# lemma-osu/sknnr

Hardware: AMD Instinct MI355X
Metric: Mqueries/sec + achieved HBM GB/s, 10M×50k×32 k=5, 1/2/4/8 MI355X (higher is better)
Workload: dtype f16 split MFMA (hi.hi swept, lo.hi + hi.lo corrections; f32 accumulate) pre-filter + f64 exact re-score

## Files before the change

sknnr_amd/csrc/bucket.hip.h:

```cpp
#pragma once
#include <hip/hip_runtime.h>
#include <stdint.h>

namespace sknnr {

constexpr int kCellMaxDepth = 6;
constexpr int kCellMax = 1 << kCellMaxDepth;
constexpr int kBucketBlock = 1024;
#ifndef SKNNR_BUCKET_CHUNKS
#define SKNNR_BUCKET_CHUNKS 32
#endif
constexpr int kBucketChunks = SKNNR_BUCKET_CHUNKS;

struct CellTreeDev {
    const float* axes;
    const float* centre;
    const float* thr;
    int depth;
};

__device__ __forceinline__ int cell_of(const float (&z)[kCellMaxDepth], const CellTreeDev& t) {
    int node = 0;
#pragma unroll
    for (int l = 0; l < kCellMaxDepth; ++l)
        if (l < t.depth) node = 2 * node + (z[l] >= t.thr[(1 << l) - 1 + node] ? 1 : 0);
    return node;
}

struct CellArgs {
    const double* xq;
    long nq;
    long n_pad;
    int d;
    int depth;
    const float* axes;
    const float* centre;
    const float* thr;
    unsigned char* cell;
    int* hist;
    int* perm;
    const double* qnc;
    double* qnc_pos;
};

#ifdef SKNNR_KERNELS_EXACT
__global__ void __launch_bounds__(256) cell_assign_kernel(CellArgs a) {
    const long q = (long)blockIdx.x * 256 + threadIdx.x;
    if (q < a.nq) {
        const double* row = a.xq + q * a.d;
        float z[kCellMaxDepth];
#pragma unroll
        for (int l = 0; l < kCellMaxDepth; ++l) z[l] = 0.f;
        auto feed = [&](int k, double x) {
            const float v = (float)x - a.centre[k];
#pragma unroll
            for (int l = 0; l < kCellMaxDepth; ++l)
                if (l < a.depth) z[l] = fmaf(v, a.axes[l * a.d + k], z[l]);
        };
        int k = 0;
        if ((a.d & 3) == 0) {
            const double2* r2 = (const double2*)row;
            for (; k + 8 <= a.d; k += 8) {
                const double2 v0 = r2[k / 2], v1 = r2[k / 2 + 1], v2 = r2[k / 2 + 2], v3 = r2[k / 2 + 3];
                feed(k, v0.x); feed(k + 1, v0.y); feed(k + 2, v1.x); feed(k + 3, v1.y);
                feed(k + 4, v2.x); feed(k + 5, v2.y); feed(k + 6, v3.x); feed(k + 7, v3.y);
            }
        }
        for (; k < a.d; ++k) feed(k, row[k]);
        const CellTreeDev t{a.axes, a.centre, a.thr, a.depth};
        a.cell[q] = (unsigned char)cell_of(z, t);
    }
}
#endif

#ifdef SKNNR_KERNELS_EXACT
__global__ void __launch_bounds__(kBucketBlock) cell_count_kernel(CellArgs a) {
    __shared__ int h[kCellMax];
    if (threadIdx.x < kCellMax) h[threadIdx.x] = 0;
    __syncthreads();
#pragma unroll
    for (int r = 0; r < kBucketChunks; ++r) {
        const long q = ((long)blockIdx.x * kBucketChunks + r) * kBucketBlock + threadIdx.x;
        if (q < a.nq) atomicAdd(&h[a.cell[q]], 1);
    }
    __syncthreads();
    if (threadIdx.x < kCellMax && h[threadIdx.x] != 0) atomicAdd(&a.hist[threadIdx.x], h[threadIdx.x]);
}
#endif


#ifdef SKNNR_KERNELS_EXACT
__global__ void __launch_bounds__(kBucketBlock) cell_scatter_kernel(CellArgs a) {
    __shared__ int cnt[kCellMax], base[kCellMax], first[kCellMax];
    const int n_cells = 1 << a.depth;
    if (threadIdx.x < kCellMax) cnt[threadIdx.x] = 0;
    if (threadIdx.x == 0) {
        int acc = 0;
        for (int c = 0; c < kCellMax; ++c) {
            first[c] = acc;
            acc += c < n_cells ? a.hist[c] : 0;
        }
    }
    __syncthreads();
    int c[kBucketChunks], ticket[kBucketChunks];
#pragma unroll
    for (int r = 0; r < kBucketChunks; ++r) {
        const long q = ((long)blockIdx.x * kBucketChunks + r) * kBucketBlock + threadIdx.x;
        c[r] = 0;
        ticket[r] = 0;
        if (q < a.nq) {
            c[r] = a.cell[q];
            ticket[r] = atomicAdd(&cnt[c[r]], 1);
        } else if (q < a.n_pad) {
            a.perm[q] = (int)q;
            if (a.qnc_pos) a.qnc_pos[q] = a.qnc[q];
            a.cell[q] = (unsigned char)(n_cells - 1);
        }
    }
    __syncthreads();
    if (threadIdx.x < kCellMax && cnt[threadIdx.x] != 0) base[threadIdx.x] = atomicAdd(&a.hist[kCellMax + threadIdx.x], cnt[threadIdx.x]);
    __syncthreads();
#pragma unroll
    for (int r = 0; r < kBucketChunks; ++r) {
        const long q = ((long)blockIdx.x * kBucketChunks + r) * kBucketBlock + threadIdx.x;
        if (q < a.nq) {
            const int p = first[c[r]] + base[c[r]] + ticket[r];
            a.perm[p] = (int)q;
            if (a.qnc_pos) a.qnc_pos[p] = a.qnc[q];
        }
    }
}
#endif

}
```

sknnr_amd/csrc/k_exact.hip:

```cpp
#define SKNNR_KERNELS_EXACT 1
#include <cstdint>
#include <cstdlib>

#include "launch.hip.h"

namespace sknnr {
namespace {
__global__ void add_counter_kernel(const int* __restrict__ cnt, long long* __restrict__ total) { *total += *cnt; }

template <int BT>
hipError_t prep_lds_bt(const PrepArgs& a, hipStream_t st) {
    const size_t sh = (size_t)BT * (a.d_in | 1) * 8;
    hipError_t e = hipFuncSetAttribute((const void*)prep_queries_kernel<BT>, hipFuncAttributeMaxDynamicSharedMemorySize, (int)sh);
    if (e != hipSuccess) return e;
    prep_queries_kernel<BT><<<dim3((unsigned)(a.nq_pad / BT)), dim3(BT), sh, st>>>(a);
    return hipGetLastError();
}

template <int FORMULA>
hipError_t exact_scan_f(bool chunked, const ScanArgs& a, long blocks, size_t sh, hipStream_t st) {
    auto kern = chunked ? exact_scan_kernel<FORMULA, true> : exact_scan_kernel<FORMULA, false>;
    hipError_t e = hipFuncSetAttribute((const void*)kern, hipFuncAttributeMaxDynamicSharedMemorySize, (int)sh);
    if (e != hipSuccess) return e;
    kern<<<dim3((unsigned)blocks), dim3(kScanWaves * 64), sh, st>>>(a);
    return hipGetLastError();
}
}

namespace launch {

hipError_t row_norms(const double* x, long n, int d, double* out, hipStream_t st) {
    row_norms_kernel<<<dim3((unsigned)((n + 255) / 256)), dim3(256), 0, st>>>(x, n, d, out);
    return hipGetLastError();
}

template <int KS>
hipError_t prep_direct_ks(PrepArgs a, hipStream_t st) {
    a.lds_wave_bytes = prep_direct_wave_lds(KS, a.xt != nullptr, a.qimg != nullptr);
    const size_t sh = (size_t)4 * a.lds_wave_bytes;
    hipError_t e = hipFuncSetAttribute((const void*)prep_queries_direct_kernel<KS>, hipFuncAttributeMaxDynamicSharedMemorySize, (int)sh);
    if (e != hipSuccess) return e;
    prep_queries_direct_kernel<KS><<<dim3((unsigned)(a.nq_pad / 256)), dim3(256), sh, st>>>(a);
    return hipGetLastError();
}

hipError_t prep_direct(const PrepArgs& a, hipStream_t st) {
    switch (a.ks) {
        case 1: return prep_direct_ks<1>(a, st);
        case 2: return prep_direct_ks<2>(a, st);
        case 3: return prep_direct_ks<3>(a, st);
        case 4: return prep_direct_ks<4>(a, st);
    }
    return hipErrorInvalidValue;
}

hipError_t prep_lds(int rows_per_block, const PrepArgs& a, hipStream_t st) {
    switch (rows_per_block) {
        case 256: return prep_lds_bt<256>(a, st);
        case 128: return prep_lds_bt<128>(a, st);
        case 64: return prep_lds_bt<64>(a, st);
    }
    return hipErrorInvalidValue;
}

hipError_t check_finite(const double* x, long n_el, int* status, hipStream_t st) {
    const long blocks = n_el + 255 < 256L * 256 * 16 ? (n_el + 255) / 256 : 256L * 16;
    check_finite_kernel<<<dim3((unsigned)(blocks < 1 ? 1 : blocks)), dim3(256), 0, st>>>(x, n_el, status);
    return hipGetLastError();
}

hipError_t cell_assign(const CellArgs& a, hipStream_t st) {
    cell_assign_kernel<<<dim3((unsigned)((a.nq + 255) / 256)), dim3(256), 0, st>>>(a);
    return hipGetLastError();
}
hipError_t cell_count(const CellArgs& a, hipStream_t st) {
    cell_count_kernel<<<dim3((unsigned)((a.nq + kBucketBlock * kBucketChunks - 1) / (kBucketBlock * kBucketChunks))), dim3(kBucketBlock), 0, st>>>(a);
    return hipGetLastError();
}
hipError_t cell_scatter(const CellArgs& a, hipStream_t st) {
    cell_scatter_kernel<<<dim3((unsigned)((a.n_pad + kBucketBlock * kBucketChunks - 1) / (kBucketBlock * kBucketChunks))), dim3(kBucketBlock), 0, st>>>(a);
    return hipGetLastError();
}

int finalize_lanes(const FinalizeArgs& f) { return f.rec ? kRecordLen : (f.m_list <= 8 ? 16 : (f.m_list <= 16 ? 32 : 64)); }

hipError_t finalize(const FinalizeArgs& f, long n, hipStream_t st) {
    if (f.rec) {
        finalize_record_kernel<<<dim3((unsigned)((n * kRecordLen + 255) / 256)), dim3(256), finalize_lds_bytes(kRecordLen / 2, f.s.d), st>>>(f);
    } else if (f.m_list <= 8) {
        finalize_kernel<8><<<dim3((unsigned)((n * 16 + 255) / 256)), dim3(256), finalize_lds_bytes(8, f.s.d), st>>>(f);
    } else if (f.m_list <= 16) {
        finalize_kernel<16><<<dim3((unsigned)((n * 32 + 255) / 256)), dim3(256), finalize_lds_bytes(16, f.s.d), st>>>(f);
    } else {
        finalize_kernel<32><<<dim3((unsigned)((n * 64 + 255) / 256)), dim3(256), finalize_lds_bytes(32, f.s.d), st>>>(f);
    }
    return hipGetLastError();
}

hipError_t exact_scan(int formula, bool chunked, const ScanArgs& a, long blocks, size_t lds_bytes, hipStream_t st) {
    switch (formula) {
        case 0: return exact_scan_f<0>(chunked, a, blocks, lds_bytes, st);
        case 1: return exact_scan_f<1>(chunked, a, blocks, lds_bytes, st);
        default: return exact_scan_f<2>(chunked, a, blocks, lds_bytes, st);
    }
}

hipError_t scan_merge(int formula, const ScanArgs& a, long blocks, size_t lds_bytes, int grid_wg_of_scan, int forced_slices,
                      hipStream_t st) {
    const dim3 grid((unsigned)blocks), block(256);
    switch (formula) {
        case 0: scan_merge_kernel<0><<<grid, block, lds_bytes, st>>>(a, grid_wg_of_scan, forced_slices); break;
        case 1: scan_merge_kernel<1><<<grid, block, lds_bytes, st>>>(a, grid_wg_of_scan, forced_slices); break;
        default: scan_merge_kernel<2><<<grid, block, lds_bytes, st>>>(a, grid_wg_of_scan, forced_slices); break;
    }
    return hipGetLastError();
}

hipError_t pack_shards(const double* val, const long* idx, long nq, int n_shards, int kk, double* slice_v, int* slice_i,
                       hipStream_t st) {
    const long heaps = nq * n_shards * kk;
    const long blocks = (heaps + 255) / 256 < 256L * 32 ? (heaps + 255) / 256 : 256L * 32;
    pack_shards_kernel<<<dim3((unsigned)(blocks < 1 ? 1 : blocks)), dim3(256), 0, st>>>(val, idx, nq, n_shards, kk, slice_v, slice_i);
    return hipGetLastError();
}

hipError_t predict(const PredictArgs& a, hipStream_t st) {
    const long total = a.nq * a.t;
    if ((a.mode == 0 && a.y32) || (a.mode == 2 && a.w32))
        predict32_kernel<<<dim3((unsigned)((total + 255) / 256)), dim3(256), 0, st>>>(a);
    else if (a.k <= 8)
        predict_kernel<<<dim3((unsigned)((total + 255) / 256)), dim3(256), 0, st>>>(a);
    else
        predict_wide_kernel<<<dim3((unsigned)((total + 255) / 256)), dim3(256), 0, st>>>(a);
// ... 39 lines not shown
```

sknnr_amd/csrc/launch.hip.h:

```cpp
#pragma once
#include <hip/hip_runtime.h>

#include <algorithm>

#include "bucket.hip.h"
#include "coarse2.hip.h"
#include "exact.hip.h"
#include "forest.hip.h"
#include "hamming.hip.h"
#include "mask.hip.h"
#include "narrow.hip.h"
#include "planes.hip.h"
#include "rescue.hip.h"
#include "summary.hip.h"

namespace sknnr {
namespace launch {

hipError_t row_norms(const double* x, long n, int d, double* out, hipStream_t st);
hipError_t prep_direct(const PrepArgs& a, hipStream_t st);
hipError_t prep_lds(int rows_per_block, const PrepArgs& a, hipStream_t st);
hipError_t check_finite(const double* x, long n_el, int* status, hipStream_t st);
hipError_t cell_assign(const CellArgs& a, hipStream_t st);
hipError_t cell_count(const CellArgs& a, hipStream_t st);
hipError_t cell_scatter(const CellArgs& a, hipStream_t st);
hipError_t finalize(const FinalizeArgs& f, long n, hipStream_t st);
int finalize_lanes(const FinalizeArgs& f);
hipError_t exact_scan(int formula, bool chunked, const ScanArgs& a, long blocks, size_t lds_bytes, hipStream_t st);
hipError_t scan_merge(int formula, const ScanArgs& a, long blocks, size_t lds_bytes, int grid_wg_of_scan, int forced_slices,
                      hipStream_t st);
hipError_t pack_shards(const double* val, const long* idx, long nq, int n_shards, int kk, double* slice_v, int* slice_i,
                       hipStream_t st);
hipError_t predict(const PredictArgs& a, hipStream_t st);
hipError_t crosswalk(const long* table, const long* idx, long n, long* out, hipStream_t st);
hipError_t add_counter(const int* cnt, long long* total, hipStream_t st);
hipError_t rescue(int ks, const RescueArgs& a, hipStream_t st);
hipError_t rescue_account(const int* listed, const int* state, long long* total, hipStream_t st);

hipError_t hamming_pack(const double* xq, long nq, long nq_pad, int t, int tp, uint32_t* qimg, int* q_bad, hipStream_t st);
hipError_t hamming_rows(const double* x, long n, int t, int tpr, uint32_t* rows, hipStream_t st);
hipError_t hamming_coarse(const HammingArgs& a, hipStream_t st);
hipError_t hamming_rescore(const HammingRescoreArgs& a, hipStream_t st);
hipError_t hamming_distance_rows(const HammingRowsArgs& a, hipStream_t st);

hipError_t forest_apply(const ForestArgs& a, hipStream_t st);

hipError_t row_mask(const MaskArgs& a, long* n_valid, hipStream_t st);
hipError_t row_compact(const CompactArgs& a, size_t row_bytes, hipStream_t st);
int compact_unit(const void* x, const void* out, size_t row_bytes);
hipError_t row_expand(const ExpandArgs& a, hipStream_t st);

hipError_t planes_to_rows(const PlanesArgs& a, int elem_bytes, hipStream_t st);
hipError_t rows_to_planes(const PlanesArgs& a, hipStream_t st);

hipError_t narrow(const NarrowArgs& a, int kind, int dst_dtype, bool wide, hipStream_t st);
int narrow_dst_bytes(int kind, int dst_dtype);

hipError_t summary(const SummaryArgs& a, hipStream_t st);

struct Coarse1Launch {
    const char* rimg;
    int n_stages;
    const uint4* qimg;
    const double* qnc;
    float skip_scale;
    int n_sentinel;
    float* cand_val;
    int* cand_idx;
    long nq_pad;
};
struct Coarse2Launch {
    const char* rhi;
    const char* rlo;
    int n_stages;
    const uint4* qimg;
    const double* qnc;
    float skip_scale;
// ... 21 lines not shown
```

sknnr_amd/csrc/sknnr_hip.hip:

```cpp
#include "../../include/sknnr_hip.h"

#include <hip/hip_runtime.h>
#include <sys/mman.h>

#include <algorithm>
#include <chrono>
#include <cmath>
#include <cstdarg>
#include <cstdio>
#include <cstdlib>
#include <condition_variable>
#include <cstring>
#include <deque>
#include <functional>
#include <future>
#include <limits>
#include <memory>
#include <mutex>
#include <new>
#include <string>
#include <thread>
#include <vector>

#include "launch.hip.h"
// ... 181 lines not shown
                q_.pop_front();
            }
            task();
        }
    }
    std::mutex m_;
    std::condition_variable cv_;
    std::deque<std::packaged_task<int()>> q_;
    bool stop_ = false;
    std::thread th_;
};

struct sknnr_index {
    int device = 0;
    long n_ref = 0;
    int d = 0, t = 0;
    int ks = 0;
    int n_stages = 0;
    double s = 1.0;
    double ymax = 0.0;
    double mu_norm = 0.0;
    std::vector<double> mu;
    std::mutex mtx;

    int d_in = 0;
    bool has_affine = false;
    DevBuf<double> center, scale, proj;
    bool has_center = false, has_scale = false, has_proj = false;

    bool has_forest = false;
    int f_d_in = 0;
    DevBuf<int4> f_nodes;
    DevBuf<long> f_off;
    DevBuf<int> f_depth;
    DevBuf<double> f_ids;

    DevBuf<double> hw;
    double hw_sum = 0.0;
    bool has_hw = false;
    bool h16_ok = false;
    int h_tp = 0, h_ref_pad = 0;
    DevBuf<uint32_t> h_rimg, h_wq, h_qimg, h_rrow;
    DevBuf<int> h_bad, h_cand_cnt, h_cand_id;
    DevBuf<double> ref64, refT, rn64, y64, mu_dev;
    DevBuf<char> rimg;
    DevBuf<char> rhi2, rlo2;
    int n_stages2 = 0;
    DevBuf<int> perm;
    DevBuf<int> perm2;
    int cell_depth = 0;
    DevBuf<float> cell_axes, cell_centre, cell_thr;
    DevBuf<int> cell_stage;
    DevBuf<unsigned char> qcell;
    DevBuf<int> qperm, cell_hist;

    DevBuf<double> xt, qnc, xstage, dist_stage, pred_stage;
    DevBuf<uint4> qimg;
    DevBuf<float> cand_val;
    DevBuf<int> cand_idx, fail_list, fail_count, fail_list2, slice_i;
    DevBuf<unsigned long long> rec;
    DevBuf<float> rec_bound;
    DevBuf<double> qnc_pos;
    DevBuf<double> slice_v;
    DevBuf<float> fail_thr;
    DevBuf<int> resc_list, resc_state;
    bool rescue_enabled = true;
    int64_t last_rescue[2] = {};
    DevBuf<int> status;
    DevBuf<long long> fail_total;
    DevBuf<long> idx_stage;

    struct HostSlot {
        double* pin_x = nullptr;  size_t pin_x_n = 0;
        double* pin_d = nullptr;  size_t pin_d_n = 0;
        long* pin_i = nullptr;    size_t pin_i_n = 0;
        double* pin_p = nullptr;  size_t pin_p_n = 0;
        DevBuf<double> dev_x, dev_d, dev_p;
        DevBuf<long> dev_i;
        DevBuf<double> dev_xp, dev_dp, dev_pp;
        DevBuf<long> dev_ip;
        DevBuf<unsigned long long> nar_i, nar_d, nar_p;
        hipEvent_t ev_h2d = nullptr, ev_done = nullptr, ev_d2h = nullptr;
        MaskBufs mask;
    } slot[kHostSlots];
    hipStream_t st_h2d = nullptr, st_run = nullptr, st_d2h = nullptr;
    std::unique_ptr<HostWorker> w_in, w_out;

    hipEvent_t ev_ws = nullptr;
    bool ws_busy = false;
    hipStream_t st_side = nullptr;
    hipEvent_t ev_fork = nullptr, ev_join = nullptr;
    long bulk_rows_done = 0;
    hipEvent_t ev_bulk_end = nullptr;
    int64_t last_prefilter[8] = {};
    int64_t last_finalize[2] = {};
    int64_t last_hamming[8] = {};
    long last_hamming_rows = 0;
    int64_t last_scan[8] = {};
    int64_t last_prep[8] = {};
    const double* last_prep_xt = nullptr;
    bool last_prep_bucketed = false, last_prep_qnc_pos = false;
    bool stream_open = false;
    MaskBufs mask;
    DevBuf<double> m_nodata, s_nodata;
    int64_t last_mask[8] = {};
    int64_t last_planes[8] = {};
    DevBuf<double> s_scale, s_offset;
    int64_t last_narrow[8] = {};
    const SummaryPlan* summary = nullptr;
    DevBuf<int> c_stat, s_stat;
    int64_t last_summary[8] = {};

    struct CallTiming {
        hipEvent_t e0 = nullptr, e1 = nullptr;
        std::vector<std::pair<hipEvent_t, hipEvent_t>> coarse;
        size_t coarse_used = 0;
        long coarse_rows = 0;
        bool pending = false;
    };
    static constexpr int kTimingRing = 64;
    CallTiming timing[kTimingRing];
    int timing_next = 0;
    sknnr_stats stats{};

    ~sknnr_index() {
        w_in.reset();
        w_out.reset();
        (void)hipSetDevice(device);
        for (auto* b : {&center, &scale, &proj, &ref64, &refT, &rn64, &y64, &mu_dev, &xt, &qnc, &xstage,
                        &dist_stage, &pred_stage, &f_ids})
            b->release();
        f_nodes.release(); f_off.release(); f_depth.release();
        rimg.release();
        perm.release();
        perm2.release();
        cell_axes.release(); cell_centre.release(); cell_thr.release(); cell_stage.release();
        qcell.release(); qperm.release(); cell_hist.release();
        h_rimg.release(); h_wq.release(); h_qimg.release(); h_rrow.release(); h_bad.release(); h_cand_cnt.release(); h_cand_id.release();
        qimg.release();
        cand_val.release();
        cand_idx.release();
        rec.release(); rec_bound.release(); qnc_pos.release();
        fail_list.release();
        fail_count.release();
        fail_thr.release(); resc_list.release(); resc_state.release();
        fail_total.release();
        status.release();
        idx_stage.release();
        for (auto& sl : slot) {
            for (void* hp : {(void*)sl.pin_x, (void*)sl.pin_d, (void*)sl.pin_i, (void*)sl.pin_p})
                if (hp) (void)hipHostFree(hp);
            sl.dev_x.release(); sl.dev_d.release(); sl.dev_p.release(); sl.dev_i.release();
            sl.dev_xp.release(); sl.dev_dp.release(); sl.dev_pp.release(); sl.dev_ip.release();
            sl.nar_i.release(); sl.nar_d.release(); sl.nar_p.release();
            for (hipEvent_t e : {sl.ev_h2d, sl.ev_done, sl.ev_d2h})
                if (e) (void)hipEventDestroy(e);
        }
        for (hipStream_t h : {st_h2d, st_run, st_d2h})
            if (h) (void)hipStreamDestroy(h);
        if (ev_ws) (void)hipEventDestroy(ev_ws);
        if (st_side) (void)hipStreamDestroy(st_side);
        for (hipEvent_t e : {ev_fork, ev_join})
            if (e) (void)hipEventDestroy(e);
        for (auto& ct : timing) {
            for (hipEvent_t e : {ct.e0, ct.e1})
                if (e) (void)hipEventDestroy(e);
            for (auto& pr : ct.coarse) {
                (void)hipEventDestroy(pr.first);
                (void)hipEventDestroy(pr.second);
            }
        }
    }
};

extern "C" int32_t sknnr_device_count(void) {
    int n = 0;
    if (hipGetDeviceCount(&n) != hipSuccess) return 0;
    return n;
}

extern "C" int32_t sknnr_abi_version(void) { return SKNNR_ABI_VERSION; }

extern "C" const char* sknnr_last_error(void) { return g_last_error.c_str(); }

extern "C" int sknnr_index_shape(const sknnr_index* ix, int64_t* n_ref, int32_t* d, int32_t* t,
                                 int32_t* d_in, int32_t* device) {
    if (!ix) return fail(SKNNR_ERR_INVALID, "index is NULL");
    if (n_ref) *n_ref = ix->n_ref;
    if (d) *d = ix->d;
    if (t) *t = ix->t;
    if (d_in) *d_in = ix->has_affine ? ix->d_in : (ix->has_forest ? ix->f_d_in : ix->d);
    if (device) *device = ix->device;
    return SKNNR_OK;
}

static bool mahalanobis_norms(const double* ref, int64_t n_ref, int d, const std::vector<double>& mu,
                              std::vector<double>& out) {
    if ((double)n_ref * d * d > 8e9 || n_ref < 2 * (int64_t)d) return false;
// ... 404 lines not shown
                    std::vector<int> first_s((size_t)n_cells + 1, sim.S);
                    for (int pos = sim.S - 1; pos >= 0; --pos) first_s[(size_t)tree.code[(size_t)by_cell[(size_t)pos]]] = pos;
                    for (int c = n_cells - 1; c >= 0; --c)
                        if (first_s[(size_t)c] == sim.S) first_s[(size_t)c] = first_s[(size_t)c + 1];
                    const int window = std::max<int>(32, (int)((int64_t)seed_tiles_for(n_tiles2, tps2) * 32 * sim.S / n_ref));
                    std::vector<int> start((size_t)sim.NQ);
                    for (int qi = 0; qi < sim.NQ; ++qi) {
                        int node = 0;
                        for (int l = 0; l < depth; ++l) {
                            float z = 0.f;
                            for (int k = 0; k < d; ++k)
                                z = std::fmaf((float)sim.q[(size_t)qi * d + k] - tree.centre[(size_t)k], tree.axes[(size_t)l * d + k], z);
                            node = 2 * node + (z >= tree.thr[((size_t)1 << l) - 1 + node] ? 1 : 0);
                        }
                        const int mid = (first_s[(size_t)node] + first_s[(size_t)node + 1]) / 2;
                        start[(size_t)qi] = ((mid - window / 2) % sim.S + sim.S) % sim.S;
                    }
                    const long v_cell = sim.visits(by_cell, &start);
                    if (v_cell * 100 >= order_visits * 85) depth = 0;
                    if (std::getenv("SKNNR_ORDER_TRACE"))
                        std::fprintf(stderr, "[order] best plain order %d: %ld visits; cell order (depth %d): %ld visits -> %s\n", image_order,
                                     order_visits, tree.depth, v_cell, depth ? "cells" : "plain");
                }
            }
            if (depth > 0) {
                for (int64_t i = 0; i < n_ref; ++i) perm2[(size_t)i] = (int)i;
                const bool by_norm = std::getenv("SKNNR_CELL_NORM_ORDER") != nullptr;
                std::stable_sort(perm2.begin(), perm2.end(), [&](int a, int b) {
                    if (tree.code[(size_t)a] != tree.code[(size_t)b]) return tree.code[(size_t)a] < tree.code[(size_t)b];
                    if (by_norm) return cnorm[(size_t)a] < cnorm[(size_t)b];
                    return mix((uint32_t)a) < mix((uint32_t)b);
                });
                const int n_cells = 1 << depth;
                std::vector<long> first((size_t)n_cells + 1, n_ref);
                for (int64_t pos = n_ref - 1; pos >= 0; --pos) first[(size_t)tree.code[(size_t)perm2[(size_t)pos]]] = pos;
                for (int c = n_cells - 1; c >= 0; --c)
                    if (first[(size_t)c] == n_ref) first[(size_t)c] = first[(size_t)c + 1];
                std::vector<int> stage((size_t)n_cells);
                for (int c = 0; c < n_cells; ++c) {
                    const long mid_tile = (first[(size_t)c] + first[(size_t)c + 1]) / 2 / 32;
                    const long half = seed_tiles_for(n_tiles2, tps2) / 2;
                    long st = (mid_tile - half) / tps2;
                    if (mid_tile - half < 0) st = ix->n_stages2 + (mid_tile - half - tps2 + 1) / tps2;
                    stage[(size_t)c] = (int)(((st % ix->n_stages2) + ix->n_stages2) % ix->n_stages2);
                }
                HIP_TRY(ix->cell_axes.ensure(tree.axes.size()));
                HIP_TRY(hipMemcpy(ix->cell_axes.p, tree.axes.data(), tree.axes.size() * sizeof(float), hipMemcpyHostToDevice));
                HIP_TRY(ix->cell_centre.ensure(tree.centre.size()));
                HIP_TRY(hipMemcpy(ix->cell_centre.p, tree.centre.data(), tree.centre.size() * sizeof(float), hipMemcpyHostToDevice));
                HIP_TRY(ix->cell_thr.ensure(tree.thr.size()));
                HIP_TRY(hipMemcpy(ix->cell_thr.p, tree.thr.data(), tree.thr.size() * sizeof(float), hipMemcpyHostToDevice));
                HIP_TRY(ix->cell_stage.ensure(stage.size()));
                HIP_TRY(hipMemcpy(ix->cell_stage.p, stage.data(), stage.size() * sizeof(int), hipMemcpyHostToDevice));
                HIP_TRY(ix->cell_hist.ensure(2 * kCellMax));
                ix->cell_depth = depth;
            }
            const size_t tb2 = tile2_bytes(ks), lob = (size_t)ks * 1024;
            std::vector<char> hi2(n_tiles2 * tb2, 0), lo2(n_tiles2 * lob, 0);
            for (long tile = 0; tile < n_tiles2; ++tile)
                fill_tile(perm2, tile, reinterpret_cast<uint16_t*>(hi2.data() + tile * tb2),
                          reinterpret_cast<uint16_t*>(lo2.data() + tile * lob), reinterpret_cast<float*>(hi2.data() + tile * tb2 + lob));
            HIP_TRY(ix->rhi2.ensure(hi2.size()));
            HIP_TRY(hipMemcpy(ix->rhi2.p, hi2.data(), hi2.size(), hipMemcpyHostToDevice));
            HIP_TRY(ix->rlo2.ensure(lo2.size()));
            HIP_TRY(hipMemcpy(ix->rlo2.p, lo2.data(), lo2.size(), hipMemcpyHostToDevice));
            HIP_TRY(ix->perm2.ensure((size_t)n_ref));
            HIP_TRY(hipMemcpy(ix->perm2.p, perm2.data(), (size_t)n_ref * sizeof(int), hipMemcpyHostToDevice));
        }
        {
            double m2 = 0.0;
            for (int c = 0; c < d; ++c) m2 += ix->mu[c] * ix->mu[c];
            ix->mu_norm = std::sqrt(m2) * (1.0 + 1e-12);
        }
        HIP_TRY(ix->rimg.ensure(img.size()));
        HIP_TRY(hipMemcpy(ix->rimg.p, img.data(), img.size(), hipMemcpyHostToDevice));
        HIP_TRY(ix->perm.ensure((size_t)n_ref));
        HIP_TRY(hipMemcpy(ix->perm.p, perm.data(), (size_t)n_ref * sizeof(int), hipMemcpyHostToDevice));
        HIP_TRY(ix->mu_dev.ensure(dp));
        HIP_TRY(hipMemcpy(ix->mu_dev.p, ix->mu.data(), dp * sizeof(double), hipMemcpyHostToDevice));
    }

    HIP_TRY(ix->fail_count.ensure(4));
    HIP_TRY(ix->resc_state.ensure(kRescueWords));
    {
        const char* e = std::getenv("SKNNR_RESCUE");
        ix->rescue_enabled = !(e && std::atoi(e) == 0);
    }
    HIP_TRY(ix->fail_total.ensure(2));
    HIP_TRY(hipMemset(ix->fail_total.p, 0, 16));
    HIP_TRY(ix->status.ensure(4));
    HIP_TRY(hipMemset(ix->status.p, 0, 16));
    HIP_TRY(hipEventCreateWithFlags(&ix->ev_ws, hipEventDisableTiming));
    HIP_TRY(hipDeviceSynchronize());
    guard.p = nullptr;
    *out = ix;
    return SKNNR_OK;
}

extern "C" void sknnr_index_destroy(sknnr_index* ix) { delete ix; }

extern "C" int sknnr_index_set_affine(sknnr_index* ix, int32_t d_in, const double* center,
                                      const double* scale, const double* proj) {
    if (!ix) return fail(SKNNR_ERR_INVALID, "index is NULL");
    if (d_in < 1) return fail(SKNNR_ERR_INVALID, "d_in must be >= 1");
    if (!proj && d_in != ix->d)
        return fail(SKNNR_ERR_INVALID, "without a projection d_in (%d) must equal d (%d)", d_in, ix->d);
    std::lock_guard<std::mutex> lock(ix->mtx);
    HIP_TRY(hipSetDevice(ix->device));
    HIP_TRY(hipDeviceSynchronize());
    ix->d_in = d_in;
    ix->has_center = center != nullptr;
    ix->has_scale = scale != nullptr;
    ix->has_proj = proj != nullptr;
    if (center) {
        HIP_TRY(ix->center.ensure(d_in));
        HIP_TRY(hipMemcpy(ix->center.p, center, d_in * sizeof(double), hipMemcpyHostToDevice));
    }
    if (scale) {
        HIP_TRY(ix->scale.ensure(d_in));
        HIP_TRY(hipMemcpy(ix->scale.p, scale, d_in * sizeof(double), hipMemcpyHostToDevice));
    }
    if (proj) {
        const int dp = ix->ks > 0 ? 16 * ix->ks : ((ix->d + 15) / 16) * 16;
        std::vector<double> padded((size_t)d_in * dp, 0.0);
        for (int c = 0; c < d_in; ++c)
            for (int j = 0; j < ix->d; ++j) padded[(size_t)c * dp + j] = proj[(size_t)c * ix->d + j];
        HIP_TRY(ix->proj.ensure(padded.size()));
        HIP_TRY(hipMemcpy(ix->proj.p, padded.data(), padded.size() * sizeof(double), hipMemcpyHostToDevice));
    }
    ix->has_affine = true;
    return SKNNR_OK;
}

extern "C" int sknnr_index_set_hamming_weights(sknnr_index* ix, const double* w, int32_t n) {
    if (!ix) return fail(SKNNR_ERR_INVALID, "index is NULL");
    if (!w || n != ix->d) return fail(SKNNR_ERR_INVALID, "w must hold one weight per column (%d), got %d", ix->d, n);
// ... 511 lines not shown
    if (o->n_neighbors + (o->exclude_self ? 1 : 0) > kScanMaxKK)
        return fail(SKNNR_ERR_UNSUPPORTED, "n_neighbors = %d exceeds the HIP backend's limit of %d%s", o->n_neighbors,
                    kScanMaxKK - (o->exclude_self ? 1 : 0),
                    o->exclude_self ? " with X=None (the query rows' own rows are searched too)" : "");
    if (std::abs(o->decimals) > 300) return fail(SKNNR_ERR_INVALID, "decimals out of range");
    return SKNNR_OK;
}

int run_forest(sknnr_index* ix, const void* xdev, long nq, const sknnr_query_opts* o, double* d_dist, long* d_idx,
               hipStream_t st);
void zero_records(sknnr_index* ix) {
    std::fill(std::begin(ix->last_prefilter), std::end(ix->last_prefilter), 0);
    std::fill(std::begin(ix->last_hamming), std::end(ix->last_hamming), 0);
    std::fill(std::begin(ix->last_finalize), std::end(ix->last_finalize), 0);
    std::fill(std::begin(ix->last_scan), std::end(ix->last_scan), 0);
    std::fill(std::begin(ix->last_rescue), std::end(ix->last_rescue), 0);
    std::fill(std::begin(ix->last_prep), std::end(ix->last_prep), 0);
    std::fill(std::begin(ix->last_mask), std::end(ix->last_mask), 0);
    ix->last_hamming_rows = 0;
}
int run_device(sknnr_index* ix, const void* xdev, long nq, const sknnr_query_opts* o, double* d_dist,
               long* d_idx, hipStream_t st, int raw = 0, long id_offset = 0) {
    zero_records(ix);
    if (xdev && uses_forest(ix, o)) return run_forest(ix, xdev, nq, o, d_dist, d_idx, st);
    const int kk = o->n_neighbors + (o->exclude_self ? 1 : 0);
    const bool affine = o->apply_affine != 0 && xdev != nullptr;
    const bool self_rows = xdev == nullptr;
    const int x_dtype = self_rows ? kDtypeF64 : o->query_dtype;
    const bool to_xt = affine || x_dtype != kDtypeF64;
    static const bool scan_everything = std::getenv("SKNNR_EXACT_ONLY") != nullptr;
    const bool coarse = ix->ks > 0 && kk <= kCoarseMaxKK && o->formula != SKNNR_FORMULA_HAMMING && !scan_everything;
    const int d_x = affine ? ix->d_in : ix->d;
    if (nq > 0x7fffffffL) return fail(SKNNR_ERR_UNSUPPORTED, "more than 2^31 - 1 query rows in one call");
    if (affine && ix->ks == 0)
        return fail(SKNNR_ERR_UNSUPPORTED, "d = %d > 128 with an affine map is outside the HIP envelope", ix->d);
    if (ix->ws_busy) HIP_TRY(hipStreamWaitEvent(st, ix->ev_ws, 0));
    const bool check_finite = o->check_finite != 0 && xdev != nullptr;

    const double* xq_call = self_rows ? ix->ref64.p + o->row_offset * ix->d : (const double*)xdev;
    if (to_xt) {
        HIP_TRY(ix->xt.ensure((size_t)nq * ix->d));
        xq_call = ix->xt.p;
    }
    const long chunk = chunk_rows(ix->ks, coarse_list_len(ix, kk));
    const long cap = std::min(chunk, nq);
    const long cap_pad = (cap + kRowQuantum - 1) / kRowQuantum * kRowQuantum;
    if (coarse || to_xt) {
        HIP_TRY(ix->qimg.ensure((size_t)(cap_pad / 32) * 2 * ix->ks * 64));
        HIP_TRY(ix->qnc.ensure(cap_pad));
    }
    if (coarse && ix->cell_depth > 0) {
        HIP_TRY(ix->qcell.ensure((size_t)cap_pad));
        HIP_TRY(ix->qperm.ensure((size_t)cap_pad));
    }
    const bool record = coarse && use_record(ix->ks, coarse_list_len(ix, kk), kk, use_coarse2(ix, coarse_list_len(ix, kk)), raw);
    if (record) {
        HIP_TRY(ix->rec.ensure((size_t)cap_pad * kRecordLen));
        HIP_TRY(ix->rec_bound.ensure((size_t)cap_pad));
        if (ix->cell_depth > 0) HIP_TRY(ix->qnc_pos.ensure((size_t)cap_pad));
    } else if (coarse) {
        HIP_TRY(ix->cand_val.ensure((size_t)cap_pad * 2 * coarse_list_len(ix, kk)));
        HIP_TRY(ix->cand_idx.ensure((size_t)cap_pad * 2 * coarse_list_len(ix, kk)));
    }
    if (coarse) {
        HIP_TRY(ix->fail_list.ensure(nq));
        HIP_TRY(hipMemsetAsync(ix->fail_count.p, 0, 16, st));
    }
    const bool rescue = coarse && ix->rescue_enabled && !raw && kk <= kRescueMaxKK && use_coarse2(ix, coarse_list_len(ix, kk));
    if (rescue) {
        HIP_TRY(ix->fail_thr.ensure(nq));
        HIP_TRY(ix->resc_list.ensure(nq));
        HIP_TRY(hipMemsetAsync(ix->resc_state.p, 0, kRescueWords * sizeof(int), st));
        ix->last_rescue[0] = 1;
        ix->last_rescue[1] = ix->ks;
    }

    SelectArgs call{};
    call.xq = xq_call;
    call.ref = ix->ref64.p;
    call.rn = ix->rn64.p;
    call.nq = nq;
    call.d = ix->d;
    call.n_ref = (int)ix->n_ref;
    call.k = o->n_neighbors;
    call.kk = kk;
    call.exclude_self = o->exclude_self ? 1 : 0;
    call.deterministic = o->deterministic ? 1 : 0;
    call.formula = o->formula;
    call.pow10_is_divisor = o->decimals < 0;
    call.pow10 = std::pow(10.0, std::abs(o->decimals));
    call.row_offset = o->row_offset;
    call.hw = ix->hw.p;
    call.hw_sum = ix->hw_sum;
    call.raw = raw;
    call.id_offset = id_offset;
    if (raw) call.deterministic = 0;
    call.out_dist = d_dist;
    call.out_idx = d_idx;

    sknnr_index::CallTiming& ct = ix->timing[ix->timing_next];
    ix->timing_next = (ix->timing_next + 1) % sknnr_index::kTimingRing;
    resolve_call(ix, ct);
    if (!ct.e0) {
        HIP_TRY(hipEventCreate(&ct.e0));
        HIP_TRY(hipEventCreate(&ct.e1));
    }
    ct.coarse_used = 0;
    ct.coarse_rows = 0;
    HIP_TRY(hipEventRecord(ct.e0, st));
    if (check_finite && !(coarse || to_xt)) {
        const long n_el = nq * (long)d_x;
        HIP_TRY(launch::check_finite((const double*)xdev, n_el, ix->status.p, st));
    }
    for (long c0 = 0; c0 < nq; c0 += chunk) {
        const long n = std::min(chunk, nq - c0);
        const long n_pad = (n + kRowQuantum - 1) / kRowQuantum * kRowQuantum;
        const void* xin = self_rows ? (const void*)(xq_call + c0 * ix->d)
                                    : (const void*)((const char*)xdev + (size_t)c0 * d_x * dtype_bytes(x_dtype));
        const bool bucketed = coarse && ix->cell_depth > 0 && use_coarse2(ix, coarse_list_len(ix, kk));
        bool cells_done = false;
        if (coarse || to_xt) {
            int rc = launch_prep(ix, xin, n, n_pad, affine, to_xt ? ix->xt.p + c0 * ix->d : nullptr, st, check_finite, bucketed, &cells_done,
                                 x_dtype);
            if (rc) return rc;
        }
        if (!coarse) continue;

        if (ct.coarse_used == ct.coarse.size()) {
            hipEvent_t e0, e1;
            HIP_TRY(hipEventCreate(&e0));
            HIP_TRY(hipEventCreate(&e1));
            ct.coarse.emplace_back(e0, e1);
        }
        auto& ev = ct.coarse[ct.coarse_used++];
        const bool v2 = use_coarse2(ix, coarse_list_len(ix, kk));
        if (bucketed) {
            CellArgs ca{};
            ca.xq = xq_call + c0 * ix->d;
            ca.nq = n;
            ca.n_pad = n_pad;
            ca.d = ix->d;
            ca.depth = ix->cell_depth;
            ca.axes = ix->cell_axes.p;
            ca.centre = ix->cell_centre.p;
            ca.thr = ix->cell_thr.p;
            ca.cell = ix->qcell.p;
            ca.hist = ix->cell_hist.p;
            ca.perm = ix->qperm.p;
            ca.qnc = ix->qnc.p;
            ca.qnc_pos = record ? ix->qnc_pos.p : nullptr;
            HIP_TRY(hipMemsetAsync(ix->cell_hist.p, 0, 2 * kCellMax * sizeof(int), st));
            if (!cells_done) HIP_TRY(launch::cell_assign(ca, st));
            HIP_TRY(launch::cell_count(ca, st));
            HIP_TRY(launch::cell_scatter(ca, st));
            if (!cells_done) ix->last_prep[6] = 2;
            ix->last_prep_bucketed = true;
            ix->last_prep_qnc_pos = record;
        }
        HIP_TRY(hipEventRecord(ev.first, st));
        if (v2 && !ix->st_side && !std::getenv("SKNNR_NO_SIDE_STREAM")) {
            HIP_TRY(hipStreamCreateWithFlags(&ix->st_side, hipStreamNonBlocking));
            HIP_TRY(hipEventCreateWithFlags(&ix->ev_fork, hipEventDisableTiming));
            HIP_TRY(hipEventCreateWithFlags(&ix->ev_join, hipEventDisableTiming));
        }
        ix->bulk_rows_done = 0;
        ix->ev_bulk_end = ev.second;
        std::fill(std::begin(ix->last_prefilter), std::end(ix->last_prefilter), 0);
        ix->last_prefilter[7] = bucketed ? ix->cell_depth : 0;
        {
            const long tiles = v2 ? (long)ix->n_stages2 * tiles_per_stage2(ix->ks) +
                                        seed_tiles_for((long)ix->n_stages2 * tiles_per_stage2(ix->ks), tiles_per_stage2(ix->ks))
                                  : (long)ix->n_stages * tiles_per_stage(ix->ks);
            ix->stats.mfma_executed_ratio = (double)tiles * 32.0 * (16.0 * ix->ks) / ((double)ix->n_ref * ix->d);
        }
        int rc = v2 ? launch_coarse2(ix, n, coarse_list_len(ix, kk), kk, record, st)
                    : launch_coarse(ix, n_pad, coarse_list_len(ix, kk), kk, st);
        if (rc) return rc;
        if (ix->ev_bulk_end) HIP_TRY(hipEventRecord(ev.second, st));
        ix->ev_bulk_end = nullptr;
        ct.coarse_rows += ix->bulk_rows_done > 0 ? std::min<long>(ix->bulk_rows_done, n) : n;

        FinalizeArgs f{};
        f.s = call;
        f.s.xq = xq_call + c0 * ix->d;
        f.s.nq = n;
        f.s.row_offset = o->row_offset + c0;
        f.s.out_dist = d_dist ? d_dist + c0 * o->n_neighbors : nullptr;
        f.s.out_idx = d_idx + c0 * o->n_neighbors;
        f.cand_val = ix->cand_val.p;
        f.cand_idx = ix->cand_idx.p;
        f.perm = v2 ? ix->perm2.p : ix->perm.p;
        f.qnc = ix->qnc.p;
        f.qperm = bucketed ? ix->qperm.p : nullptr;
        if (record) {
            f.rec = ix->rec.p;
            f.rec_bound = ix->rec_bound.p;
            f.qnc_pos = bucketed ? ix->qnc_pos.p : ix->qnc.p;
            f.trunc_count = ix->fail_count.p + 3;
        }
        f.m_list = coarse_list_len(ix, kk);
        f.rank_extra = coarse_rank_extra(f.m_list, kk);
        f.inv_s2 = 1.0 / (ix->s * ix->s);
        f.s2 = ix->s * ix->s;
        f.inv_s = 1.0 / ix->s;
        f.eps_c = (v2 ? eps_units2(ix->ks) : eps_units(ix->ks)) * std::ldexp(1.0, -24);
        f.ymax = ix->ymax;
// ... 1970 lines not shown
```

Measured before the change: 230.8.

## Make query cell bucketing a deterministic stable counting sort with per-block histograms

Replaces the atomic-ticket bucket scatter with a three-pass counting sort. Per-block cell histograms are built from vectorized 16-byte cell loads with run-length atomics, a single-block kernel computes exclusive prefix offsets, and the scatter uses wave ballots to rank same-cell lanes, sorting locally in LDS before writing perm coalesced. Control words (fail count, rescue state, cell hist) are merged into one buffer so a single memset replaces three. This removes global atomics and scattered writes from bucketing, at the cost of an extra serial one-block scan launch and more LDS per block.

```diff
diff --git a/sknnr_amd/csrc/bucket.hip.h b/sknnr_amd/csrc/bucket.hip.h
--- a/sknnr_amd/csrc/bucket.hip.h
+++ b/sknnr_amd/csrc/bucket.hip.h
@@ -6,11 +6,10 @@
 
 constexpr int kCellMaxDepth = 6;
 constexpr int kCellMax = 1 << kCellMaxDepth;
-constexpr int kBucketBlock = 1024;
-#ifndef SKNNR_BUCKET_CHUNKS
-#define SKNNR_BUCKET_CHUNKS 32
-#endif
-constexpr int kBucketChunks = SKNNR_BUCKET_CHUNKS;
+constexpr int kBucketBlock = 256;
+constexpr int kBucketRounds = 16;
+constexpr int kBucketRows = kBucketBlock * kBucketRounds;
+constexpr int kBucketScanThreads = 1024;
 
 struct CellTreeDev {
     const float* axes;
@@ -38,6 +37,8 @@
     const float* thr;
     unsigned char* cell;
     int* hist;
+    int* block_hist;
+    int n_blocks;
     int* perm;
     const double* qnc;
     double* qnc_pos;
@@ -75,59 +76,175 @@
 
 #ifdef SKNNR_KERNELS_EXACT
 __global__ void __launch_bounds__(kBucketBlock) cell_count_kernel(CellArgs a) {
+    static_assert(kBucketRounds == 16, "one 16-byte load of cells per thread");
     __shared__ int h[kCellMax];
     if (threadIdx.x < kCellMax) h[threadIdx.x] = 0;
     __syncthreads();
-#pragma unroll
-    for (int r = 0; r < kBucketChunks; ++r) {
-        const long q = ((long)blockIdx.x * kBucketChunks + r) * kBucketBlock + threadIdx.x;
-        if (q < a.nq) atomicAdd(&h[a.cell[q]], 1);
-    }
-    __syncthreads();
-    if (threadIdx.x < kCellMax && h[threadIdx.x] != 0) atomicAdd(&a.hist[threadIdx.x], h[threadIdx.x]);
+    const long q0 = (long)blockIdx.x * kBucketRows + (long)threadIdx.x * kBucketRounds;
+    if (q0 + kBucketRounds <= a.nq) {
+        const uint4 v = *reinterpret_cast<const uint4*>(a.cell + q0);
+        const unsigned w[4] = {v.x, v.y, v.z, v.w};
+        int run_cell = (int)(w[0] & 255u), run = 0;
+#pragma unroll
+        for (int r = 0; r < kBucketRounds; ++r) {
+            const int c = (int)((w[r >> 2] >> (8 * (r & 3))) & 255u);
+            if (c != run_cell) {
+                atomicAdd(&h[run_cell], run);
+                run_cell = c;
+                run = 0;
+            }
+            ++run;
+        }
+        atomicAdd(&h[run_cell], run);
+    } else {
+        for (int r = 0; r < kBucketRounds; ++r)
+            if (q0 + r < a.nq) atomicAdd(&h[a.cell[q0 + r]], 1);
+    }
+    __syncthreads();
+    if (threadIdx.x < kCellMax) a.block_hist[(long)blockIdx.x * kCellMax + threadIdx.x] = h[threadIdx.x];
+}
+
+__global__ void __launch_bounds__(kBucketScanThreads) cell_scan_kernel(CellArgs a) {
+    constexpr int kSeg = kBucketScanThreads / kCellMax;
+    __shared__ int seg[kSeg][kCellMax];
+    __shared__ int first[kCellMax];
+    const int c = threadIdx.x % kCellMax, s = threadIdx.x / kCellMax;
+    const int len = (a.n_blocks + kSeg - 1) / kSeg;
+    const int b0 = s * len, b1 = b0 + len < a.n_blocks ? b0 + len : a.n_blocks;
+    int* col = a.block_hist + c;
+    int sum = 0;
+    int b = b0;
+    for (; b + 4 <= b1; b += 4) {
+        const int v0 = col[(long)b * kCellMax], v1 = col[(long)(b + 1) * kCellMax], v2 = col[(long)(b + 2) * kCellMax],
+                  v3 = col[(long)(b + 3) * kCellMax];
+        sum += (v0 + v1) + (v2 + v3);
+    }
+    for (; b < b1; ++b) sum += col[(long)b * kCellMax];
+    seg[s][c] = sum;
+    __syncthreads();
+    if (s == 0) {
+        int acc = 0;
+        for (int t = 0; t < kSeg; ++t) {
+            const int v = seg[t][c];
+            seg[t][c] = acc;
+            acc += v;
+        }
+        a.hist[c] = acc;
+        first[c] = acc;
+    }
+    __syncthreads();
+    if (threadIdx.x == 0) {
+        int acc = 0;
+        for (int t = 0; t < kCellMax; ++t) {
+            const int v = first[t];
+            first[t] = acc;
+            acc += v;
+        }
+    }
+    __syncthreads();
+    int run = first[c] + seg[s][c];
+    b = b0;
+    for (; b + 4 <= b1; b += 4) {
+        const int v0 = col[(long)b * kCellMax], v1 = col[(long)(b + 1) * kCellMax], v2 = col[(long)(b + 2) * kCellMax],
+                  v3 = col[(long)(b + 3) * kCellMax];
+        col[(long)b * kCellMax] = run;
+        col[(long)(b + 1) * kCellMax] = run + v0;
+        col[(long)(b + 2) * kCellMax] = run + v0 + v1;
+        col[(long)(b + 3) * kCellMax] = run + v0 + v1 + v2;
+        run += (v0 + v1) + (v2 + v3);
+    }
+    for (; b < b1; ++b) {
+        const int v = col[(long)b * kCellMax];
+        col[(long)b * kCellMax] = run;
+        run += v;
+    }
 }
 #endif
 
+__device__ __forceinline__ unsigned long long same_cell_lanes(int c, bool live, int depth) {
+    unsigned long long m = __ballot(live);
+#pragma unroll
+    for (int l = 0; l < kCellMaxDepth; ++l)
+        if (l < depth) {
+            const bool bit = (c >> l) & 1;
+            const unsigned long long set = __ballot(bit);
+            m &= bit ? set : ~set;
+        }
+    return m;
+}
 
 #ifdef SKNNR_KERNELS_EXACT
 __global__ void __launch_bounds__(kBucketBlock) cell_scatter_kernel(CellArgs a) {
-    __shared__ int cnt[kCellMax], base[kCellMax], first[kCellMax];
+    constexpr int kWaves = kBucketBlock / 64;
+    __shared__ int start[kWaves][kCellMax];
+    __shared__ int first[kCellMax];
+    __shared__ unsigned sorted[kBucketRows];
     const int n_cells = 1 << a.depth;
-    if (threadIdx.x < kCellMax) cnt[threadIdx.x] = 0;
-    if (threadIdx.x == 0) {
-        int acc = 0;
-        for (int c = 0; c < kCellMax; ++c) {
-            first[c] = acc;
-            acc += c < n_cells ? a.hist[c] : 0;
-        }
-    }
-    __syncthreads();
-    int c[kBucketChunks], ticket[kBucketChunks];
-#pragma unroll
-    for (int r = 0; r < kBucketChunks; ++r) {
-        const long q = ((long)blockIdx.x * kBucketChunks + r) * kBucketBlock + threadIdx.x;
-        c[r] = 0;
-        ticket[r] = 0;
-        if (q < a.nq) {
-            c[r] = a.cell[q];
-            ticket[r] = atomicAdd(&cnt[c[r]], 1);
-        } else if (q < a.n_pad) {
+    const int lane = threadIdx.x & 63, wave = threadIdx.x >> 6;
+    const unsigned long long below = (1ull << lane) - 1ull;
+    for (int i = threadIdx.x; i < kWaves * kCellMax; i += kBucketBlock) (&start[0][0])[i] = 0;
+    __syncthreads();
+    volatile int* mine = start[wave];
+    const long qb = (long)blockIdx.x * kBucketRows;
+    const int r0 = wave * (kBucketRounds * 64) + lane;
+#pragma unroll 1
+    for (int r = 0; r < kBucketRounds; ++r) {
+        const long q = qb + r0 + r * 64;
+        if (q - lane >= a.nq) break;
+        const bool live = q < a.nq;
+        const int c = live ? a.cell[q] : 0;
+        const unsigned long long m = same_cell_lanes(c, live, a.depth);
+        if (live && (m & below) == 0) mine[c] = mine[c] + __popcll(m);
+    }
+    __syncthreads();
+    if (threadIdx.x < kCellMax) {
+        int total = 0;
+#pragma unroll
+        for (int w = 0; w < kWaves; ++w) total += start[w][threadIdx.x];
+        int before = total;
+#pragma unroll
+        for (int sh = 1; sh < kCellMax; sh <<= 1) {
+            const int v = __shfl_up(before, sh);
+            if ((int)threadIdx.x >= sh) before += v;
+        }
+        int acc = before - total;
+        first[threadIdx.x] = a.block_hist[(long)blockIdx.x * kCellMax + threadIdx.x] - acc;
+#pragma unroll
+        for (int w = 0; w < kWaves; ++w) {
+            const int v = start[w][threadIdx.x];
+            start[w][threadIdx.x] = acc;
+            acc += v;
+        }
+    }
+    __syncthreads();
+#pragma unroll 1
+    for (int r = 0; r < kBucketRounds; ++r) {
+        const int rb = r0 + r * 64;
+        const long q = qb + rb;
+        if (q - lane >= a.n_pad) break;
+        const bool live = q < a.nq;
+        if (!live && q < a.n_pad) {
             a.perm[q] = (int)q;
             if (a.qnc_pos) a.qnc_pos[q] = a.qnc[q];
             a.cell[q] = (unsigned char)(n_cells - 1);
         }
-    }
-    __syncthreads();
-    if (threadIdx.x < kCellMax && cnt[threadIdx.x] != 0) base[threadIdx.x] = atomicAdd(&a.hist[kCellMax + threadIdx.x], cnt[threadIdx.x]);
-    __syncthreads();
-#pragma unroll
-    for (int r = 0; r < kBucketChunks; ++r) {
-        const long q = ((long)blockIdx.x * kBucketChunks + r) * kBucketBlock + threadIdx.x;
-        if (q < a.nq) {
-            const int p = first[c[r]] + base[c[r]] + ticket[r];
-            a.perm[p] = (int)q;
-            if (a.qnc_pos) a.qnc_pos[p] = a.qnc[q];
-        }
+        const int c = live ? a.cell[q] : 0;
+        const unsigned long long m = same_cell_lanes(c, live, a.depth);
+        if (live) {
+            const int at = mine[c];
+            if ((m & below) == 0) mine[c] = at + __popcll(m);
+            sorted[at + __popcll(m & below)] = (unsigned)c << 16 | (unsigned)rb;
+        }
+    }
+    __syncthreads();
+    const long left = a.nq - qb;
+    const int n_live = left >= kBucketRows ? kBucketRows : (left > 0 ? (int)left : 0);
+    for (int i = threadIdx.x; i < n_live; i += kBucketBlock) {
+        const unsigned e = sorted[i];
+        const long q = qb + (e & 0xffffu);
+        const int p = first[e >> 16] + i;
+        a.perm[p] = (int)q;
+        if (a.qnc_pos) a.qnc_pos[p] = a.qnc[q];
     }
 }
 #endif
diff --git a/sknnr_amd/csrc/k_exact.hip b/sknnr_amd/csrc/k_exact.hip
--- a/sknnr_amd/csrc/k_exact.hip
+++ b/sknnr_amd/csrc/k_exact.hip
@@ -74,11 +74,15 @@
     return hipGetLastError();
 }
 hipError_t cell_count(const CellArgs& a, hipStream_t st) {
-    cell_count_kernel<<<dim3((unsigned)((a.nq + kBucketBlock * kBucketChunks - 1) / (kBucketBlock * kBucketChunks))), dim3(kBucketBlock), 0, st>>>(a);
+    cell_count_kernel<<<dim3((unsigned)a.n_blocks), dim3(kBucketBlock), 0, st>>>(a);
+    return hipGetLastError();
+}
+hipError_t cell_scan(const CellArgs& a, hipStream_t st) {
+    cell_scan_kernel<<<dim3(1), dim3(kBucketScanThreads), 0, st>>>(a);
     return hipGetLastError();
 }
 hipError_t cell_scatter(const CellArgs& a, hipStream_t st) {
-    cell_scatter_kernel<<<dim3((unsigned)((a.n_pad + kBucketBlock * kBucketChunks - 1) / (kBucketBlock * kBucketChunks))), dim3(kBucketBlock), 0, st>>>(a);
+    cell_scatter_kernel<<<dim3((unsigned)a.n_blocks), dim3(kBucketBlock), 0, st>>>(a);
     return hipGetLastError();
 }
 
diff --git a/sknnr_amd/csrc/launch.hip.h b/sknnr_amd/csrc/launch.hip.h
--- a/sknnr_amd/csrc/launch.hip.h
+++ b/sknnr_amd/csrc/launch.hip.h
@@ -23,6 +23,7 @@
 hipError_t check_finite(const double* x, long n_el, int* status, hipStream_t st);
 hipError_t cell_assign(const CellArgs& a, hipStream_t st);
 hipError_t cell_count(const CellArgs& a, hipStream_t st);
+hipError_t cell_scan(const CellArgs& a, hipStream_t st);
 hipError_t cell_scatter(const CellArgs& a, hipStream_t st);
 hipError_t finalize(const FinalizeArgs& f, long n, hipStream_t st);
 int finalize_lanes(const FinalizeArgs& f);
diff --git a/sknnr_amd/csrc/sknnr_hip.hip b/sknnr_amd/csrc/sknnr_hip.hip
--- a/sknnr_amd/csrc/sknnr_hip.hip
+++ b/sknnr_amd/csrc/sknnr_hip.hip
@@ -257,18 +257,21 @@
     DevBuf<float> cell_axes, cell_centre, cell_thr;
     DevBuf<int> cell_stage;
     DevBuf<unsigned char> qcell;
-    DevBuf<int> qperm, cell_hist;
+    DevBuf<int> qperm, block_hist;
 
     DevBuf<double> xt, qnc, xstage, dist_stage, pred_stage;
     DevBuf<uint4> qimg;
     DevBuf<float> cand_val;
-    DevBuf<int> cand_idx, fail_list, fail_count, fail_list2, slice_i;
+    DevBuf<int> cand_idx, fail_list, fail_list2, slice_i;
+    DevBuf<int> ctrl;
+    struct Words { int* p = nullptr; } fail_count, resc_state, cell_hist;
+    static constexpr size_t kCtrlWords = 4 + kRescueWords + kCellMax;
     DevBuf<unsigned long long> rec;
     DevBuf<float> rec_bound;
     DevBuf<double> qnc_pos;
     DevBuf<double> slice_v;
     DevBuf<float> fail_thr;
-    DevBuf<int> resc_list, resc_state;
+    DevBuf<int> resc_list;
     bool rescue_enabled = true;
     int64_t last_rescue[2] = {};
     DevBuf<int> status;
@@ -340,15 +343,16 @@
         perm.release();
         perm2.release();
         cell_axes.release(); cell_centre.release(); cell_thr.release(); cell_stage.release();
-        qcell.release(); qperm.release(); cell_hist.release();
+        qcell.release(); qperm.release(); block_hist.release();
         h_rimg.release(); h_wq.release(); h_qimg.release(); h_rrow.release(); h_bad.release(); h_cand_cnt.release(); h_cand_id.release();
         qimg.release();
         cand_val.release();
         cand_idx.release();
         rec.release(); rec_bound.release(); qnc_pos.release();
         fail_list.release();
-        fail_count.release();
-        fail_thr.release(); resc_list.release(); resc_state.release();
+        ctrl.release();
+        fail_count.p = resc_state.p = cell_hist.p = nullptr;
+        fail_thr.release(); resc_list.release();
         fail_total.release();
         status.release();
         idx_stage.release();
@@ -859,7 +863,6 @@
                 HIP_TRY(hipMemcpy(ix->cell_thr.p, tree.thr.data(), tree.thr.size() * sizeof(float), hipMemcpyHostToDevice));
                 HIP_TRY(ix->cell_stage.ensure(stage.size()));
                 HIP_TRY(hipMemcpy(ix->cell_stage.p, stage.data(), stage.size() * sizeof(int), hipMemcpyHostToDevice));
-                HIP_TRY(ix->cell_hist.ensure(2 * kCellMax));
                 ix->cell_depth = depth;
             }
             const size_t tb2 = tile2_bytes(ks), lob = (size_t)ks * 1024;
@@ -887,8 +890,11 @@
         HIP_TRY(hipMemcpy(ix->mu_dev.p, ix->mu.data(), dp * sizeof(double), hipMemcpyHostToDevice));
     }
 
-    HIP_TRY(ix->fail_count.ensure(4));
-    HIP_TRY(ix->resc_state.ensure(kRescueWords));
+    HIP_TRY(ix->ctrl.ensure(sknnr_index::kCtrlWords));
+    HIP_TRY(hipMemset(ix->ctrl.p, 0, sknnr_index::kCtrlWords * sizeof(int)));
+    ix->fail_count.p = ix->ctrl.p;
+    ix->resc_state.p = ix->ctrl.p + 4;
+    ix->cell_hist.p = ix->ctrl.p + 4 + kRescueWords;
     {
         const char* e = std::getenv("SKNNR_RESCUE");
         ix->rescue_enabled = !(e && std::atoi(e) == 0);
@@ -1506,6 +1512,7 @@
     if (coarse && ix->cell_depth > 0) {
         HIP_TRY(ix->qcell.ensure((size_t)cap_pad));
         HIP_TRY(ix->qperm.ensure((size_t)cap_pad));
+        HIP_TRY(ix->block_hist.ensure((size_t)((cap_pad + kBucketRows - 1) / kBucketRows) * kCellMax));
     }
     const bool record = coarse && use_record(ix->ks, coarse_list_len(ix, kk), kk, use_coarse2(ix, coarse_list_len(ix, kk)), raw);
     if (record) {
@@ -1518,13 +1525,12 @@
     }
     if (coarse) {
         HIP_TRY(ix->fail_list.ensure(nq));
-        HIP_TRY(hipMemsetAsync(ix->fail_count.p, 0, 16, st));
+        HIP_TRY(hipMemsetAsync(ix->ctrl.p, 0, sknnr_index::kCtrlWords * sizeof(int), st));
     }
     const bool rescue = coarse && ix->rescue_enabled && !raw && kk <= kRescueMaxKK && use_coarse2(ix, coarse_list_len(ix, kk));
     if (rescue) {
         HIP_TRY(ix->fail_thr.ensure(nq));
         HIP_TRY(ix->resc_list.ensure(nq));
-        HIP_TRY(hipMemsetAsync(ix->resc_state.p, 0, kRescueWords * sizeof(int), st));
         ix->last_rescue[0] = 1;
         ix->last_rescue[1] = ix->ks;
     }
@@ -1603,9 +1609,11 @@
             ca.perm = ix->qperm.p;
             ca.qnc = ix->qnc.p;
             ca.qnc_pos = record ? ix->qnc_pos.p : nullptr;
-            HIP_TRY(hipMemsetAsync(ix->cell_hist.p, 0, 2 * kCellMax * sizeof(int), st));
+            ca.block_hist = ix->block_hist.p;
+            ca.n_blocks = (int)((n_pad + kBucketRows - 1) / kBucketRows);
             if (!cells_done) HIP_TRY(launch::cell_assign(ca, st));
             HIP_TRY(launch::cell_count(ca, st));
+            HIP_TRY(launch::cell_scan(ca, st));
             HIP_TRY(launch::cell_scatter(ca, st));
             if (!cells_done) ix->last_prep[6] = 2;
             ix->last_prep_bucketed = true;
```

Result: no change. 231.5, median of 6 (+0.3%).
